# onolab-tmu/overiva

Hardware: AMD Instinct MI355X
Metric: AuxIVA iterations/sec (2048 bins x 4000 frames x 8 mics) (higher is better)
Workload: dtype f32

## Files before the change

include/overiva_hip.h:

```cpp
#ifndef OVERIVA_HIP_H
#define OVERIVA_HIP_H

#ifdef __cplusplus
extern "C" {
#endif

#define OIVA_OK 0
#define OIVA_ERR_ARG (-1)
#define OIVA_ERR_HIP (-2)
#define OIVA_ERR_STATE (-3)
#define OIVA_ERR_NUMERIC (-4)

#define OIVA_MODEL_LAPLACE 0
#define OIVA_MODEL_GAUSS 1

#define OIVA_MAX_CHANNELS 32

#define OIVA_PREC_FAST 0
#define OIVA_PREC_UPDATE_F64 1
#define OIVA_PREC_UPDATE_ROWS 2
#define OIVA_PREC_COV_F64 4
#define OIVA_PREC_PRECISE (OIVA_PREC_UPDATE_F64 | OIVA_PREC_COV_F64)

typedef struct oiva_plan oiva_plan;
// ... 28 lines not shown
int oiva_plan_demix_dev(oiva_plan *p, int proj_back, void **Y_dev);
int oiva_plan_demix_c128(oiva_plan *p, void *Y_host, long long row_pitch_bytes, int proj_back);

#define OIVA_XCHG_MAX_RANKS 16
#define OIVA_XCHG_HANDLE_BYTES 64
typedef struct oiva_xchg oiva_xchg;
int oiva_xchg_create(oiva_xchg **x, int device, int rank, int world, long long part_bytes);
int oiva_xchg_export(oiva_xchg *x, void *handle);
int oiva_xchg_connect(oiva_xchg *x, const void *handles);
int oiva_xchg_push(oiva_xchg *x, void *stream, const void *part_dev, long long part_bytes, int epoch);
int oiva_xchg_wait(oiva_xchg *x, void *stream, int epoch);
int oiva_xchg_gathered(oiva_xchg *x, int epoch, void **gathered);
int oiva_xchg_poll(oiva_xchg *x, int epoch, int timeout_ms, int *arrived);
int oiva_xchg_force(oiva_xchg *x, int epoch);
int oiva_xchg_destroy(oiva_xchg *x);

int oiva_plan_set_w_pca(oiva_plan *p, double *evals_host);
int oiva_plan_set_w_eig(oiva_plan *p);
int oiva_plan_get_w(oiva_plan *p, void *W_host, int f64);

int oiva_plan_sync(oiva_plan *p);
int oiva_plan_save_w(oiva_plan *p);
int oiva_plan_restore_w(oiva_plan *p);

int oiva_plan_iterate_timed(oiva_plan *p, int n, float *total_ms, float *per_kernel_ms);
#define OIVA_N_STAGES 4

int oiva_plan_get_cov_splits(oiva_plan *p, int *nsplit);
int oiva_plan_set_cov_splits(oiva_plan *p, int nsplit);
int oiva_plan_set_cov_quad(oiva_plan *p, int enable, int *active);
int oiva_plan_set_pow_splits(oiva_plan *p, int nsplit);
int oiva_plan_set_cov_hmfma(oiva_plan *p, int enable);
int oiva_plan_set_fuse_cov_update(oiva_plan *p, int enable, int *active);
int oiva_plan_use_graph(oiva_plan *p, int enable);
int oiva_plan_set_precision(oiva_plan *p, int flags);

struct oiva_xchg;
#define OIVA_RESIDENT_INFO 12
#define OIVA_RESIDENT_PHASES 8
int oiva_plan_set_resident(oiva_plan *p, int enable);
int oiva_plan_resident_info(oiva_plan *p, int *info );
int oiva_plan_resident_phases(oiva_plan *p, double *phase_us , int *n_iter);
int oiva_plan_resident_debug(oiva_plan *p, int timeout_ms, int stall_block);
int oiva_plan_resident_debug_from(oiva_plan *p, int timeout_ms, int stall_block, int first_stalled_iteration);
int oiva_plan_resident_loopback(oiva_plan *p, int world);
#define OIVA_RESIDENT_STAMPS 16
int oiva_plan_resident_trace(oiva_plan *p, int enable, unsigned long long *stamps_host, int *n_wg, int *n_iter);
int oiva_plan_resident_connect(oiva_plan *p, struct oiva_xchg *x);
int oiva_plan_fused_connect(oiva_plan *p, struct oiva_xchg *x);
int oiva_plan_fused_loopback(oiva_plan *p, int world);
int oiva_plan_fused_debug(oiva_plan *p, int timeout_ms, int stall);
int oiva_plan_set_resident_splits(oiva_plan *p, int nsplit);

int oiva_test_set_rinv(oiva_plan *p, const float *rinv_host );
int oiva_test_get_rinv(oiva_plan *p, float *rinv_host , float *wscale_host );
int oiva_test_run_weighted_cov(oiva_plan *p);
int oiva_test_get_v(oiva_plan *p, void *V_host , int f64);
int oiva_test_run_update(oiva_plan *p);
int oiva_test_get_what(oiva_plan *p, void *What_host , int f64);
int oiva_test_set_what(oiva_plan *p, const void *What_host, int f64);
int oiva_test_run_power(oiva_plan *p, float *p_host );
int oiva_test_time_stage(oiva_plan *p, int stage, int reps, float *avg_ms);

#define OIVA_OGIVE_DEMIX 0
#define OIVA_OGIVE_MIX 1
#define OIVA_OGIVE_SWITCHING 2
int oiva_plan_ogive_begin(oiva_plan *p, int update_mode, int model);
int oiva_plan_ogive_iterate(oiva_plan *p, int first_epoch, int n, double step_size, double tol, int *epochs_run,
                            int *converged, double *max_delta);

typedef struct oiva_batch oiva_batch;
int oiva_batch_create(oiva_batch **out, int device, int B, int T, int F, int M, int K, int model, void *stream);
int oiva_batch_destroy(oiva_batch *b);
int oiva_batch_set_x_host(oiva_batch *b, const void *X_host, int f64);
int oiva_batch_set_x_dev(oiva_batch *b, const void *X_dev);
int oiva_batch_covariance(oiva_batch *b);
int oiva_batch_set_w(oiva_batch *b, const void *W0_host, int f64);
int oiva_batch_set_w_eig(oiva_batch *b);
int oiva_batch_iterate(oiva_batch *b, int n);
int oiva_batch_demix(oiva_batch *b, void *Y_host, int f64, int proj_back);
int oiva_batch_get_w(oiva_batch *b, void *W_host, int f64);
int oiva_batch_status(oiva_batch *b, int *status);
int oiva_batch_time_stages(oiva_batch *b, int n, float *total_ms, float *per_stage_ms);

typedef int oiva_status;
oiva_status oiva_batch_get_cx(oiva_batch *b, void *Cx_host, int f64);
oiva_status oiva_batch_ogive_begin(oiva_batch *b, int update_mode, int model);
oiva_status oiva_batch_ogive_iterate(oiva_batch *b, int first_epoch, int n, double step_size, double tol, int *epochs_run,
                                     int *converged, double *max_delta);

oiva_status oiva_batch_create_ragged(oiva_batch **out, int device, int B, const int *frames, int F, int M, int K, int model,
                                     void *stream);

typedef struct oiva_stft oiva_stft;
// ... 23 lines not shown
```

overiva_amd/_lib.py:

```python
import ctypes as C
import os

import numpy as np

_PKG = os.path.dirname(os.path.abspath(__file__))
LIB_PATH = os.environ.get("OIVA_LIB") or os.path.join(_PKG, "liboveriva_hip.so")

OK, ERR_ARG, ERR_HIP, ERR_STATE, ERR_NUMERIC = 0, -1, -2, -3, -4
MODEL_IDS = {"laplace": 0, "gauss": 1}
N_STAGES = 4
PREC_FAST, PREC_UPDATE_F64, PREC_UPDATE_ROWS, PREC_COV_F64 = 0, 1, 2, 4
PREC_PRECISE = PREC_UPDATE_F64 | PREC_COV_F64
PREC_MIXED = PREC_UPDATE_F64
PREC_BY_NAME = {"fast": PREC_FAST, "mixed": PREC_MIXED, "precise": PREC_PRECISE}
STAGE_NAMES = ("demix_power", "activation", "weighted_cov", "ip_update")


class HipLibraryMissing(ImportError):
    pass


class HipError(RuntimeError):
    """a HIP runtime call failed inside the library"""

# ... 14 lines not shown
    "oiva_plan_set_w": [_vp, _vp, _i],
    "oiva_plan_iterate": [_vp, _i],
    "oiva_plan_power": [_vp],
    "oiva_plan_power_buffer": [_vp, _i, C.POINTER(_vp), C.POINTER(_ll)],
    "oiva_plan_update": [_vp, _vp, _i],
    "oiva_plan_demix": [_vp, _vp, _ll, _i],
    "oiva_plan_demix_dev": [_vp, _i, _vp],
    "oiva_plan_set_io_slab": [_vp, _ll],
    "oiva_host_prefault": [_vp, _ll],
    "oiva_pool_trim": [],
    "oiva_plan_demix_c128": [_vp, _vp, _ll, _i],
    "oiva_plan_set_w_pca": [_vp, _vp],
    "oiva_plan_set_w_eig": [_vp],
    "oiva_xchg_create": [_vp, _i, _i, _i, _ll],
    "oiva_xchg_export": [_vp, _vp],
    "oiva_xchg_connect": [_vp, _vp],
    "oiva_xchg_push": [_vp, _vp, _vp, _ll, _i],
    "oiva_xchg_wait": [_vp, _vp, _i],
    "oiva_xchg_gathered": [_vp, _i, _vp],
    "oiva_xchg_poll": [_vp, _i, _i, _vp],
    "oiva_xchg_force": [_vp, _i],
    "oiva_xchg_destroy": [_vp],
    "oiva_plan_get_w": [_vp, _vp, _i],
    "oiva_plan_sync": [_vp],
    "oiva_plan_save_w": [_vp],
    "oiva_plan_restore_w": [_vp],
    "oiva_plan_iterate_timed": [_vp, _i, _fp, _fp],
    "oiva_plan_get_cov_splits": [_vp, C.POINTER(_i)],
    "oiva_plan_set_cov_splits": [_vp, _i],
    "oiva_plan_set_cov_quad": [_vp, _i, C.POINTER(_i)],
    "oiva_plan_set_pow_splits": [_vp, _i],
    "oiva_plan_set_cov_hmfma": [_vp, _i],
    "oiva_plan_set_fuse_cov_update": [_vp, _i, C.POINTER(_i)],
    "oiva_plan_use_graph": [_vp, _i],
    "oiva_plan_set_precision": [_vp, _i],
    "oiva_plan_set_resident": [_vp, _i],
    "oiva_plan_resident_info": [_vp, C.POINTER(_i)],
    "oiva_plan_resident_phases": [_vp, C.POINTER(C.c_double), C.POINTER(_i)],
    "oiva_plan_resident_debug": [_vp, _i, _i],
    "oiva_plan_resident_debug_from": [_vp, _i, _i, _i],
    "oiva_plan_resident_loopback": [_vp, _i],
    "oiva_plan_fused_connect": [_vp, _vp],
    "oiva_plan_fused_loopback": [_vp, _i],
    "oiva_plan_fused_debug": [_vp, _i, _i],
    "oiva_plan_resident_connect": [_vp, _vp],
    "oiva_plan_resident_trace": [_vp, _i, _vp, C.POINTER(_i), C.POINTER(_i)],
    "oiva_plan_set_resident_splits": [_vp, _i],
    "oiva_test_set_rinv": [_vp, _vp],
    "oiva_test_get_rinv": [_vp, _vp, _vp],
    "oiva_test_run_weighted_cov": [_vp],
    "oiva_test_get_v": [_vp, _vp, _i],
    "oiva_test_run_update": [_vp],
    "oiva_test_get_what": [_vp, _vp, _i],
    "oiva_test_set_what": [_vp, _vp, _i],
    "oiva_test_run_power": [_vp, _vp],
    "oiva_test_time_stage": [_vp, _i, _i, _fp],
    "oiva_plan_ogive_begin": [_vp, _i, _i],
    "oiva_plan_ogive_iterate": [_vp, _i, _i, C.c_double, C.c_double, C.POINTER(_i), C.POINTER(_i), C.POINTER(C.c_double)],
    "oiva_batch_create": [C.POINTER(_vp), _i, _i, _i, _i, _i, _i, _i, _vp],
    "oiva_batch_destroy": [_vp],
    "oiva_batch_set_x_host": [_vp, _vp, _i],
    "oiva_batch_set_x_dev": [_vp, _vp],
    "oiva_batch_covariance": [_vp],
    "oiva_batch_set_w": [_vp, _vp, _i],
    "oiva_batch_set_w_eig": [_vp],
    "oiva_batch_iterate": [_vp, _i],
    "oiva_batch_demix": [_vp, _vp, _i, _i],
    "oiva_batch_get_w": [_vp, _vp, _i],
    "oiva_batch_status": [_vp, C.POINTER(_i)],
    "oiva_batch_time_stages": [_vp, _i, _fp, _fp],
    "oiva_batch_get_cx": [_vp, _vp, _i],
    "oiva_batch_ogive_begin": [_vp, _i, _i],
    "oiva_batch_ogive_iterate": [_vp, _i, _i, C.c_double, C.c_double, C.POINTER(_i), C.POINTER(_i), C.POINTER(C.c_double)],
    "oiva_batch_create_ragged": [C.POINTER(_vp), _i, _i, C.POINTER(_i), _i, _i, _i, _i, _vp],
    "oiva_stft_create": [C.POINTER(_vp), _i, _i, _i, _i, _i, _vp, _vp],
    "oiva_stft_destroy": [_vp],
    "oiva_stft_shape": [_vp, C.POINTER(_i), C.POINTER(_i)],
    "oiva_stft_analysis": [_vp, _vp, _vp, C.POINTER(_vp)],
    "oiva_stft_synthesis": [_vp, _vp, _i, _vp],
    "oiva_bstft_create": [C.POINTER(_vp), _i, _i, C.POINTER(_i), _i, _i, _i, _vp, _vp, _vp],
    "oiva_bstft_destroy": [_vp],
    "oiva_bstft_shape": [_vp, C.POINTER(_i), C.POINTER(_i)],
    "oiva_bstft_analysis": [_vp, _vp, C.POINTER(_vp)],
    "oiva_bstft_synthesis_dev": [_vp, _vp, _i, _vp],
    "oiva_bstft_phase_ms": [_vp, _fp],
    "oiva_batch_demix_dev": [_vp, _i, C.POINTER(_vp)],
    "oiva_device_to_host": [_vp, _vp, _ll],
}
# ... 88 lines not shown
```

overiva_amd/csrc/kernels_demix.hip:

```cpp
#include "oiva_device.h"
#include "demix_arith.h"

namespace oiva {
namespace {

constexpr int kPowUnroll = 2;

template <int M, int KP>
__global__ __launch_bounds__(kBlock) void power_kernel(const float2* __restrict__ X, const float2* __restrict__ What,
                                                       float* __restrict__ Ppart, int T, int F, int K, int tcp) {
    extern __shared__ __attribute__((aligned(16))) float sp[];
    const int tid = threadIdx.x;
    const int lane = tid & 63;
    const int wave = tid >> 6;
    const int b = lane & 15;
    const int q = lane >> 4;
    const int f = (blockIdx.x * kWaves + wave) * kBinsPerWave + b;
    const bool fvalid = f < F;
    const int fc = fvalid ? f : F - 1;
    const int k0 = blockIdx.z * KP;
    const int t_begin = blockIdx.y * tcp;
    const int t_end = min(T, t_begin + tcp);
    const int len = t_end - t_begin;
    const int nsteps = (len + 3) >> 2;

    float wr[KP][M], wi[KP][M];
    load_wconj<M, KP>(What, fc, k0, K, wr, wi);

    const size_t frame_stride = (size_t)F * M;
    const float2* pbase = X + (size_t)fc * M;
    for (int i = 0; i < nsteps; i += kPowUnroll) {
        float xr[kPowUnroll][M], xi[kPowUnroll][M];
#pragma unroll
        for (int u = 0; u < kPowUnroll; ++u) {
            const int tl = 4 * (i + u) + q;
            const int t = tl < len ? t_begin + tl : T - 1;
            load_x<M>(pbase + (size_t)t * frame_stride, xr[u], xi[u]);
        }
#pragma unroll
        for (int u = 0; u < kPowUnroll; ++u) {
            const int tl = 4 * (i + u) + q;
            const bool live = tl < len;
#pragma unroll
            for (int kk = 0; kk < KP; ++kk) {
                float yr, yi;
                demix_one<M>(wr[kk], wi[kk], xr[u], xi[u], yr, yi);
                float pw = fmaf(yr, yr, yi * yi);
                pw = fvalid ? pw : 0.f;
                pw = row16_sum(pw);
                if (b == 0 && live) sp[(wave * tcp + tl) * KP + kk] = pw;
            }
        }
    }
    __syncthreads();
    for (int e = tid; e < len * KP; e += kBlock) {
        const int tl = e / KP, kk = e - tl * KP;
        float s = sp[(0 * tcp + tl) * KP + kk];
#pragma unroll
        for (int w = 1; w < kWaves; ++w) s += sp[(w * tcp + tl) * KP + kk];
        if (k0 + kk < K) Ppart[((size_t)blockIdx.x * T + t_begin + tl) * K + k0 + kk] = s;
    }
}

template <int M, int KP>
// ... 82 lines not shown
                if (sd > 0.) {
                    zr = (float)(sr / sd);
                    zi = (float)(si / sd);
                }
#pragma unroll
                for (int m = 0; m < M; ++m) {
                    const float a = wr[kk][m], c = wi[kk][m];
                    wr[kk][m] = a * zr + c * zi;
                    wi[kk][m] = c * zr - a * zi;
                }
            }
        }
    }
    const size_t frame_stride = (size_t)F * M;
    const float2* px = X + ((size_t)(t_begin + q) * F + f) * M;
    for (int t = t_begin + q; t < t_end; t += 16) {
        float xr[M], xi[M];
        load_x<M>(px, xr, xi);
#pragma unroll
        for (int kk = 0; kk < KP; ++kk) {
            float yr, yi;
            demix_one<M>(wr[kk], wi[kk], xr, xi, yr, yi);
            if (k0 + kk < K) Y[((size_t)t * F + f) * K + k0 + kk] = make_float2(yr, yi);
        }
        px += 16 * frame_stride;
    }
}

template <int M, int KP>
hipError_t launch_power_one(hipStream_t s, const float2* X, const float2* What, float* Ppart, int T, int F, int K,
                            const PowGeom& g) {
    dim3 grid(g.nb, g.nsplit, (K + KP - 1) / KP);
    const size_t shmem = (size_t)kWaves * g.tcp * KP * sizeof(float);
    hipLaunchKernelGGL((power_kernel<M, KP>), grid, dim3(kBlock), shmem, s, X, What, Ppart, T, F, K, g.tcp);
    return hipGetLastError();
}

template <int M, int KP>
hipError_t launch_stats_one(hipStream_t s, const float2* X, const float2* What, float* Spart, int T, int F, int K,
                            const CovGeom& g) {
    dim3 grid(g.nbg, g.nsplit, (K + KP - 1) / KP);
    hipLaunchKernelGGL((stats_kernel<M, KP>), grid, dim3(kBlock), 0, s, X, What, Spart, T, F, K, g.tc);
    return hipGetLastError();
}

template <int M, int KP>
hipError_t launch_write_one(hipStream_t s, const float2* X, const float2* What, const float* Spart, int nsplit,
                            float2* Y, int T, int F, int K) {
    const int tc = 256;
    dim3 grid((F + kBinsPerWave - 1) / kBinsPerWave, (T + tc - 1) / tc, (K + KP - 1) / KP);
    hipLaunchKernelGGL((write_kernel<M, KP>), grid, dim3(kBlock), 0, s, X, What, Spart, nsplit, Y, T, F, K, tc);
    return hipGetLastError();
}

#define OIVA_DISPATCH_M(CALL)            \
    switch (M) {                         \
        case 1: CALL(1); break;          \
        case 2: CALL(2); break;          \
        case 3: CALL(3); break;          \
        case 4: CALL(4); break;          \
        case 5: CALL(5); break;          \
        case 6: CALL(6); break;          \
        case 7: CALL(7); break;          \
        case 8: CALL(8); break;          \
        case 9: CALL(9); break;          \
        case 10: CALL(10); break;        \
        case 11: CALL(11); break;        \
// ... 59 lines not shown
```

overiva_amd/csrc/oiva_internal.h:

```cpp
#pragma once
#include <hip/hip_runtime.h>
#include <hip/hip_ext.h>

#include <string>

#include "overiva_hip.h"

namespace oiva {

constexpr int kNarrowMax = 16;
constexpr int kWideMax = OIVA_MAX_CHANNELS;

int fail_with(int code, const std::string& msg);
int xchg_peers(oiva_xchg* x, char** peers, int* rank, int* world, size_t* slot_bytes);

constexpr int kBinsPerWave = 16;
constexpr int kPhasesPerWave = 4;
constexpr int kBlock = 256;
constexpr int kWaves = kBlock / 64;

__host__ __device__ inline int herm_pair_index(int M, int c, int d) {
    return M + 2 * (c * M - (c * (c + 1)) / 2 + (d - c - 1));
}

// ... 5 lines not shown

struct KernelTimer {
    hipEvent_t start = nullptr, stop = nullptr;
};
KernelTimer& kernel_timer();
inline void arm_kernel_timer(hipEvent_t start, hipEvent_t stop) {
    kernel_timer().start = start;
    kernel_timer().stop = stop;
}
template <typename Kern, typename... Args>
hipError_t launch_dominant(Kern kernel, dim3 grid, dim3 block, size_t shmem, hipStream_t s, Args... args) {
    KernelTimer& t = kernel_timer();
    if (t.start != nullptr) {
        hipExtLaunchKernelGGL(kernel, grid, block, (unsigned)shmem, s, t.start, t.stop, 0, args...);
        t.start = t.stop = nullptr;
    } else {
        hipLaunchKernelGGL(kernel, grid, block, shmem, s, args...);
    }
    return hipGetLastError();
}

struct CovGeom {
    int nsplit;
    int tc;
    int kc;
    int nbg;
    int hmfma = 0;
    int half16 = 0;
    int pair32 = 0;
    int pad = 0;
    int quad = 0;
    int part32 = 0;
};
struct PowGeom {
    int nb;
    int nsplit;
    int tcp;
    int kp;
};
constexpr int kPowMaxFrames = 512;

hipError_t launch_cov(hipStream_t s, const float2* X, const float2* Xpad, const float* R, float* Wt, float* wscale, int model, int raw,
                      void* Vpart, bool f64, int T, int F, int M, int K, const CovGeom& g);
hipError_t launch_pad_channels(hipStream_t s, const float2* X, float2* Xpad, long long n_tf, int M);
hipError_t launch_cov_mfma(hipStream_t s, const float2* X, const float* R, float* Wt, float* wscale, int model, int raw,
                           void* Vpart, bool f64, int T, int F, int M, int K, int nsplit, int tc);
bool cov_quad_supported(int M, int K);
int cov_quad_sources_per_pass(int K);
hipError_t launch_cov_quad(hipStream_t s, const float2* X, const float* R, float* Wt, float* wscale, int model, int raw,
                           double* Vpart, int T, int F, int M, int Mv, int K, const CovGeom& g);
hipError_t launch_cov_weights(hipStream_t s, const float* R, float* Wt, float* wscale, int model, int raw, int T, int K, int Kp);
bool cov_pair64_supported(int M);
int cov_pair64_sources_per_pass(int K);
int cov_pair64_bins_per_block();
hipError_t launch_cov_pair64(hipStream_t s, const float2* X, const float* R, float* Wt, float* wscale, int model, int raw,
                             double* Vpart, int T, int F, int M, int K, const CovGeom& g);
bool cov_pair32_supported(int M, int K);
int cov_pair32_sources_per_pass();
int cov_pair32_bins_per_block();
hipError_t launch_cov_pair32(hipStream_t s, const float2* X, const float* R, float* Wt, float* wscale, int model, int raw,
                             double* Vpart, int T, int F, int M, int K, const CovGeom& g);
bool cov_half16_supported(int M, int K);
int cov_half16_sources_per_pass(int K);
hipError_t launch_cov_half16(hipStream_t s, const float2* X, const float* R, float* Wt, float* wscale, int model, int raw,
                             double* Vpart, int T, int F, int M, int Mv, int K, const CovGeom& g);
bool cov_hmfma_supported(int M, int K);
hipError_t launch_cov_hmfma(hipStream_t s, const float2* X, const float* Wt, double* Vpart, int T, int F, int M, int Mv, int K, const CovGeom& g);
bool cov_hmfma64_supported(int M, int K);
hipError_t launch_cov_hmfma64(hipStream_t s, const float2* X, const double* Wt, double* Vpart, int T, int F, int M, int Mv, int K, const CovGeom& g);
bool cov_half16_f64_supported(int M, int K);
int cov_half16_f64_sources_per_pass(int K);
hipError_t launch_cov_half16_f64(hipStream_t s, const float2* X, const float* R, float* Wt, float* wscale, int model, int raw,
                                 double* Vpart, int T, int F, int M, int Mv, int K, const CovGeom& g);
// ... 212 lines not shown
```

overiva_amd/csrc/plan.hip:

```cpp
#include <algorithm>
#include <cmath>
#include <cstdint>
#include <cstdlib>
#include <cstring>
#include <mutex>
#include <string>
#include <vector>

#include "host_io.h"
#include "oiva_internal.h"
#include "resident.h"

using namespace oiva;

namespace {

thread_local std::string g_err;

int fail(int code, const std::string& msg) {
    g_err = msg;
    return code;
}

}
// ... 105 lines not shown
}
}

struct oiva_plan {
    int device = 0;
    int T = 0, F = 0, M = 0, K = 0, model = 0, F_total = 0;
    hipStream_t stream = nullptr;
    bool own_stream = false;

    const float2* X = nullptr;
    float2* X_owned = nullptr;
    size_t x_owned_bytes = 0, y_bytes = 0;
    float2* X_pad = nullptr;
    float2* What = nullptr;
    double2* What64 = nullptr;
    bool what64_valid = false;
    double* Cx = nullptr;
    void* Vpart = nullptr;
    float* Ppart = nullptr;
    int ppart_alloc = 0;
    float* Plocal = nullptr;
    void* Wwide = nullptr;
    float* R = nullptr;
    float* wscale = nullptr;
    float* Spart = nullptr;
    float2* Y = nullptr;
    double2* scratch_c = nullptr;
    double* scratch_p = nullptr;

    CovGeom cov{};
    bool cov_quad_on = true;
    bool cov_hmfma_on = true;
    bool fuse_cov_update = false;
    CovGeom stg{};
    PowGeom pw{};
    int n_cu = 256;
    int vpart_splits_alloc = 0;

    bool have_x = false, have_cx = false, have_w = false;
    bool pad_valid = false;
    bool wscale_pending = false;
    int raw_weights = 0;
    int prec = 0;
    bool upd_f64() const { return prec & OIVA_PREC_UPDATE_F64; }
    bool cov_f64() const { return prec & OIVA_PREC_COV_F64; }
    bool vpart_f64() const { return vpart_f64_of(cov); }
    bool vpart_f64_of(const CovGeom& g) const { return cov_f64() || M <= 8 || M > kNarrowMax || g.quad || (g.half16 && !g.part32); }
    int use_graph = 0;
    OgiveState og{};
    std::vector<void*> og_bufs;
    bool og_ready = false;
    int og_mode = 0, og_model = 0;
    hipGraphExec_t og_graph = nullptr;
    int og_graph_n = 0, og_graph_phase = -1;
    double og_graph_mu = 0., og_graph_tol = 0.;
    ResidentGeom rg{};
    bool res_ok = false;
    bool res_on = false;
    void* res_block = nullptr;
    float* res_parts = nullptr;
    float* res_psum = nullptr;
    double* res_vpart = nullptr;
    double* res_rsum = nullptr;
    float2* res_wpub = nullptr;
    unsigned* res_flags = nullptr;
    float2* res_what = nullptr;
// ... 145 lines not shown
        return;
    }
    g.nbg = ceil_div(p->F, kBinsPerWave);
    g.kc = 2;
    const int nz = ceil_div(p->K, g.kc);
    const int nsplit = std::min(16, pick_splits(p->n_cu * 4, g.nbg * nz, p->T, 128));
    g.tc = round_up(ceil_div(p->T, nsplit), 16);
    g.nsplit = ceil_div(p->T, g.tc);
    p->stg = g;
}

void choose_pow_geom(oiva_plan* p, int nsplit_req) {
    PowGeom g;
    g.nb = ceil_div(p->F, kBinsPerWave * kWaves);
    if (p->M > kNarrowMax) {
        g.kp = wide_pow_sources_per_pass(p->K);
        const int groups = g.nb * ceil_div(p->K, g.kp);
        const int nsplit = nsplit_req > 0 ? nsplit_req : pick_splits(p->n_cu * 4, groups, p->T, 16);
        g.tcp = round_up(ceil_div(p->T, nsplit), 4);
        g.nsplit = ceil_div(p->T, g.tcp);
        p->pw = g;
        return;
    }
    g.kp = pow_sources_per_pass(p->M, p->K);
    int nsplit = nsplit_req;
    if (nsplit <= 0) {
        const int per_cu_x12 = (g.kp == 1 && p->M <= 8) ? 24 : 12;
        nsplit = pick_splits(std::max(p->n_cu / 2, p->n_cu * per_cu_x12 / std::max(p->M, 1)), g.nb, p->T, 32);
    }
    int tcp = round_up(ceil_div(p->T, nsplit), 4);
    tcp = std::min(std::max(tcp, 4), kPowMaxFrames);
    g.tcp = tcp;
    g.nsplit = ceil_div(p->T, tcp);
    p->pw = g;
}

int drop_graph(oiva_plan* p) {
    while (!p->graphs.empty()) {
        hipGraphExec_t g = p->graphs.back().second;
        p->graphs.pop_back();
        HIP_TRY(hipGraphExecDestroy(g));
    }
    if (p->og_graph) {
        HIP_TRY(hipGraphExecDestroy(p->og_graph));
        p->og_graph = nullptr;
    }
    return OIVA_OK;
}

size_t vpart_floats(const oiva_plan* p, int nsplit) { return (size_t)nsplit * p->F * p->K * p->M * p->M; }

int ensure_vpart(oiva_plan* p) {
    if (p->cov.nsplit > p->vpart_splits_alloc) {
        if (p->Vpart) HIP_TRY(hipFree(p->Vpart));
        p->Vpart = nullptr;
        HIP_TRY(dev_malloc(&p->Vpart, (vpart_floats(p, p->cov.nsplit) + 2) * sizeof(double)));
        p->vpart_splits_alloc = p->cov.nsplit;
    }
    return OIVA_OK;
}

int stage_power(oiva_plan* p) {
    HIP_TRY(launch_power(p->stream, p->X, p->X_pad && p->pad_valid ? p->X_pad : nullptr, p->What, p->Ppart, p->T, p->F, p->M, p->K, p->pw));
    return OIVA_OK;
}
int stage_activation(oiva_plan* p, const float* parts, int nparts) {
    if (p->fx_on && parts == p->Ppart) {
        HIP_TRY(launch_activation_xchg(p->stream, parts, nparts, p->fx_gath, p->fx_rank, p->fx_world, p->fx_loopback ? (p->fx_stall ? 2 : 1) : 0, p->fx_nblk_own, p->fx_nblk_peer, p->fx_state + 16,
                                       p->fx_state, (long long)(p->fx_timeout_ms > 0 ? p->fx_timeout_ms : 2000) * 100000, p->R, p->T, p->K,
                                       p->model, p->F_total));
        p->raw_weights = 0;
        return OIVA_OK;
    }
    HIP_TRY(launch_activation(p->stream, parts, nparts, p->R, p->T, p->K, p->model, p->F_total));
    p->raw_weights = 0;
    return OIVA_OK;
}
int stage_cov(oiva_plan* p) {
    HIP_TRY(launch_cov(p->stream, p->X, p->X_pad, p->R, p->Wwide ? static_cast<float*>(p->Wwide) : p->Plocal , p->wscale, p->model,
                       p->raw_weights, p->Vpart, p->cov_f64(), p->T, p->F, p->M, p->K, p->cov));
    p->wscale_pending = !p->raw_weights;
    return OIVA_OK;
}
int stage_update(oiva_plan* p, bool init_only) {
    UpdateArgs a;
    a.What = p->What;
    a.What64 = p->upd_f64() ? p->What64 : nullptr;
    a.Cx = p->Cx;
    a.Vpart = p->Vpart;
    a.vpart_f64 = p->vpart_f64() ? 1 : 0;
    a.wscale = (!init_only && p->wscale_pending) ? p->wscale : nullptr;
    a.nsplit = p->cov.nsplit;
    a.T = p->T;
    a.F = p->F;
    a.M = p->M;
    a.K = p->K;
// ... 288 lines not shown
    p->T = T;
    p->F = F;
    p->M = M;
    p->K = K;
    p->model = model;
    p->F_total = F_total;
    if (stream) {
        p->stream = (hipStream_t)stream;
    } else {
        hipError_t e = hipStreamCreateWithFlags(&p->stream, hipStreamNonBlocking);
        if (e != hipSuccess) {
            delete p;
            return fail(OIVA_ERR_HIP, std::string("hipStreamCreate: ") + hipGetErrorString(e));
        }
        p->own_stream = true;
    }
    {
        hipDeviceProp_t prop;
        if (hipGetDeviceProperties(&prop, device) == hipSuccess && prop.multiProcessorCount > 0)
            p->n_cu = prop.multiProcessorCount;
    }
    if (M > 8 && M <= kNarrowMax && M % 2 == 1) {
        hipError_t ep = dev_malloc((void**)&p->X_pad, (size_t)T * F * (M + 1) * sizeof(float2));
        if (ep != hipSuccess) {
            oiva_plan_destroy(p);
            return fail(OIVA_ERR_HIP, std::string("allocation of the padded copy of X failed: ") + hipGetErrorString(ep));
        }
    }
    {
        const char* v = std::getenv("OIVA_COV_HMFMA");
        p->cov_hmfma_on = !(v && v[0] == '0');
        const char* u = std::getenv("OIVA_COV_UPDATE");
        p->fuse_cov_update = u && u[0] == '1';
    }
    choose_cov_geom(p, 0);
    choose_pow_geom(p, 0);
    choose_stats_geom(p);
    p->res_ok = resident_geometry(T, F, M, K, p->n_cu, 0, &p->rg);
    const size_t nTK = (size_t)T * K;
    const size_t nFMM = (size_t)F * M * M;
    hipError_t e = hipSuccess;
    auto alloc = [&](void** ptr, size_t bytes) {
        if (e == hipSuccess) e = dev_malloc(ptr, bytes);
    };
    alloc((void**)&p->What, nFMM * sizeof(float2));
    alloc((void**)&p->What64, nFMM * sizeof(double2));
    alloc((void**)&p->Cx, nFMM * sizeof(double));
    alloc((void**)&p->Ppart, (size_t)p->pw.nb * nTK * sizeof(float));
    p->ppart_alloc = p->pw.nb;
    alloc((void**)&p->Plocal, std::max(nTK, ((size_t)T + 1) * 32) * sizeof(float));
    if (M > kNarrowMax) alloc((void**)&p->Wwide, nTK * sizeof(double));
    alloc((void**)&p->R, r_buffer_bytes(T, K));
    if (e == hipSuccess) e = hipMemset(p->R, 0, r_buffer_bytes(T, K));
    alloc((void**)&p->wscale, (size_t)K * sizeof(float));
    alloc((void**)&p->Spart, (size_t)p->stg.nsplit * F * K * 3 * sizeof(float));
    alloc((void**)&p->scratch_c, (size_t)K * nFMM * sizeof(double2));
    alloc((void**)&p->scratch_p, std::max((size_t)K * nFMM, nTK) * sizeof(double));
    for (auto& ev : p->ev) {
        if (e == hipSuccess) e = hipEventCreate(&ev);
    }
    if (e != hipSuccess) {
        oiva_plan_destroy(p);
        return fail(OIVA_ERR_HIP, std::string("allocation failed: ") + hipGetErrorString(e));
    }
    int rc = ensure_vpart(p);
    if (rc) {
// ... 708 lines not shown
    DeviceGuard guard(p->device);
    if (enable >= 0) {
        HIP_TRY(hipStreamSynchronize(p->stream));
        int rc = drop_graph(p);
        if (rc) return rc;
        p->fuse_cov_update = enable != 0;
    }
    if (active) *active = cov_update_applies(p) ? 1 : 0;
    return OIVA_OK;
}

int oiva_plan_set_cov_hmfma(oiva_plan* p, int enable) {
    NEED(p, OIVA_ERR_ARG, "null plan");
    DeviceGuard guard(p->device);
    HIP_TRY(hipStreamSynchronize(p->stream));
    int rc = drop_graph(p);
    if (rc) return rc;
    p->cov_hmfma_on = enable != 0;
    choose_cov_geom(p, 0);
    return ensure_vpart(p);
}

int oiva_plan_set_pow_splits(oiva_plan* p, int nsplit) {
    NEED(p, OIVA_ERR_ARG, "null plan");
    NEED(nsplit >= 0 && nsplit <= p->T, OIVA_ERR_ARG, "bad split count");
    DeviceGuard guard(p->device);
    HIP_TRY(hipStreamSynchronize(p->stream));
    int rc = drop_graph(p);
    if (rc) return rc;
    choose_pow_geom(p, nsplit);
    return OIVA_OK;
}

int oiva_plan_use_graph(oiva_plan* p, int enable) {
    NEED(p, OIVA_ERR_ARG, "null plan");
    DeviceGuard guard(p->device);
    p->use_graph = enable ? 1 : 0;
    if (!enable) return drop_graph(p);
    if (p->have_x && p->have_cx && p->have_w && (p->F == p->F_total || p->fx_on)) return build_graphs(p);
    return OIVA_OK;
}

int oiva_plan_set_precision(oiva_plan* p, int flags) {
    NEED(p, OIVA_ERR_ARG, "null plan");
    NEED((flags & ~(OIVA_PREC_UPDATE_F64 | OIVA_PREC_UPDATE_ROWS | OIVA_PREC_COV_F64)) == 0, OIVA_ERR_ARG, "unknown precision flag");
    DeviceGuard guard(p->device);
    HIP_TRY(hipStreamSynchronize(p->stream));
    int rc = drop_graph(p);
    if (rc) return rc;
    if ((flags & OIVA_PREC_UPDATE_F64) && p->have_w && !p->what64_valid) {
        std::vector<double2> wh;
        if ((rc = download_what(p, wh)) || (rc = upload_what(p, wh))) return rc;
    }
    const bool cov_changed = ((flags ^ p->prec) & (OIVA_PREC_COV_F64 | ((p->M > 8 || p->cov.pair32) ? OIVA_PREC_UPDATE_F64 : 0))) != 0;
    p->prec = flags;
    if (cov_changed) {
        choose_cov_geom(p, 0);
        if ((rc = ensure_vpart(p))) return rc;
    }
    return OIVA_OK;
}

int oiva_plan_set_resident(oiva_plan* p, int enable) {
    NEED(p, OIVA_ERR_ARG, "null plan");
    if (!enable) {
        p->res_on = false;
// ... 360 lines not shown
            case 0: return stage_power(p);
            case 1: return stage_activation(p, p->Ppart, p->pw.nb);
            case 2: return cov_update_applies(p) ? stage_cov_update(p) : stage_cov(p);
            default: return cov_update_applies(p) ? OIVA_OK : stage_update(p, false);
        }
    };
    if ((rc = run())) return rc;
    HIP_TRY(hipEventRecord(p->ev[0], p->stream));
    for (int i = 0; i < reps; ++i)
        if ((rc = run())) return rc;
    HIP_TRY(hipEventRecord(p->ev[1], p->stream));
    HIP_TRY(hipEventSynchronize(p->ev[1]));
    float ms = 0.f;
    HIP_TRY(hipEventElapsedTime(&ms, p->ev[0], p->ev[1]));
    *avg_ms = ms / reps;
    return OIVA_OK;
}

int oiva_test_run_power(oiva_plan* p, float* p_host) {
    NEED(p && p_host, OIVA_ERR_ARG, "null argument");
    NEED(p->have_x && p->have_w, OIVA_ERR_STATE, "X / W not set");
    DeviceGuard guard(p->device);
    int rc = stage_power(p);
    if (rc) return rc;
    const size_t n = (size_t)p->T * p->K;
    HIP_TRY(launch_sum_parts(p->stream, p->Ppart, false, p->pw.nb, p->scratch_p, (long long)n, 1.));
    HIP_TRY(hipStreamSynchronize(p->stream));
    std::vector<double> sum(n);
    HIP_TRY(hipMemcpy(sum.data(), p->scratch_p, n * sizeof(double), hipMemcpyDeviceToHost));
    for (size_t i = 0; i < n; ++i) p_host[i] = (float)sum[i];
    return OIVA_OK;
}

}
```

overiva_amd/plan.py:

```python
import ctypes as C

import numpy as np

from . import _lib


def _is_f64(a):
    if a.dtype == np.complex128:
        return 1
    if a.dtype == np.complex64:
        return 0
    raise TypeError(f"complex64 or complex128 expected, got {a.dtype}")


class DeviceX:

    def __init__(self, ptr, shape, owner=None, host_dtype=np.complex64):
        self.ptr = int(ptr)
        self.shape = tuple(int(v) for v in shape)
        self.owner = owner
        self.dtype = np.dtype(host_dtype)
        self.ndim = 3


# ... 147 lines not shown
    def sync(self):
        _lib.check(self.lib.oiva_plan_sync(self.h))

    def save_w(self):
        _lib.check(self.lib.oiva_plan_save_w(self.h))

    def restore_w(self):
        _lib.check(self.lib.oiva_plan_restore_w(self.h))

    def cov_splits(self):
        n = C.c_int()
        _lib.check(self.lib.oiva_plan_get_cov_splits(self.h, C.byref(n)))
        return n.value

    def set_cov_splits(self, n):
        _lib.check(self.lib.oiva_plan_set_cov_splits(self.h, int(n)))

    def set_cov_quad(self, enable=True):
        a = C.c_int()
        _lib.check(self.lib.oiva_plan_set_cov_quad(self.h, 1 if enable else 0, C.byref(a)))
        return bool(a.value)

    def set_cov_hmfma(self, enable=True):
        _lib.check(self.lib.oiva_plan_set_cov_hmfma(self.h, 1 if enable else 0))

    def set_fuse_cov_update(self, enable=True):
        a = C.c_int()
        _lib.check(self.lib.oiva_plan_set_fuse_cov_update(self.h, -1 if enable is None else (1 if enable else 0), C.byref(a)))
        return bool(a.value)

    def set_pow_splits(self, n):
        _lib.check(self.lib.oiva_plan_set_pow_splits(self.h, int(n)))

    def use_graph(self, enable=True):
        _lib.check(self.lib.oiva_plan_use_graph(self.h, 1 if enable else 0))

    def set_precision(self, mode="fast", row_layout=False):
        flags = _lib.PREC_BY_NAME[mode] if isinstance(mode, str) else int(mode)
        if row_layout:
            flags |= _lib.PREC_UPDATE_ROWS
        _lib.check(self.lib.oiva_plan_set_precision(self.h, flags))

    RESIDENT_INFO = ("qualifies", "enabled", "bin_groups", "frame_splits", "frames_per_split", "frames_per_lane",
                     "frames_in_registers", "lds_bytes", "last_give_up_code", "launches", "fallbacks", "x_bytes_per_cu")
    RESIDENT_PHASES = ("demix_power", "parts", "activation", "cov_accumulate", "cov_reduce", "wait_partials", "ip_update", "wait_w")

    def set_resident(self, enable=True):
        _lib.check(self.lib.oiva_plan_set_resident(self.h, 1 if enable else 0))

    def resident_info(self):
        arr = (C.c_int * len(self.RESIDENT_INFO))()
        _lib.check(self.lib.oiva_plan_resident_info(self.h, arr))
        return dict(zip(self.RESIDENT_INFO, list(arr)))

    def resident_phases(self):
        arr = (C.c_double * len(self.RESIDENT_PHASES))()
        n = C.c_int()
        _lib.check(self.lib.oiva_plan_resident_phases(self.h, arr, C.byref(n)))
        return dict(zip(self.RESIDENT_PHASES, list(arr))), n.value

    def set_resident_splits(self, nsplit=0):
        _lib.check(self.lib.oiva_plan_set_resident_splits(self.h, int(nsplit)))

    def resident_connect(self, xchg_handle):
        _lib.check(self.lib.oiva_plan_resident_connect(self.h, xchg_handle))

# ... 29 lines not shown
    def t_get_rinv(self):
        r = np.empty((self.T, self.K), np.float32)
        w = np.empty((self.K,), np.float32)
        _lib.check(self.lib.oiva_test_get_rinv(self.h, _lib.ptr(r), _lib.ptr(w)))
        return r, w

    def t_run_weighted_cov(self):
        _lib.check(self.lib.oiva_test_run_weighted_cov(self.h))

    def t_get_v(self, dtype=np.complex64):
        v = np.empty((self.K, self.F, self.M, self.M), dtype)
        _lib.check(self.lib.oiva_test_get_v(self.h, _lib.ptr(v), _is_f64(v)))
        return v

    def t_run_update(self):
        _lib.check(self.lib.oiva_test_run_update(self.h))

    def t_get_what(self, dtype=np.complex64):
        w = np.empty((self.F, self.M, self.M), dtype)
        _lib.check(self.lib.oiva_test_get_what(self.h, _lib.ptr(w), _is_f64(w)))
        return w

    def t_set_what(self, What):
        What = np.asarray(What)
        What = np.ascontiguousarray(What, dtype=np.complex64 if What.dtype == np.complex64 else np.complex128)
        assert What.shape == (self.F, self.M, self.M)
        _lib.check(self.lib.oiva_test_set_what(self.h, _lib.ptr(What), _is_f64(What)))

    def t_time_stage(self, stage, reps=20):
        ms = C.c_float()
        _lib.check(self.lib.oiva_test_time_stage(self.h, _lib.STAGE_NAMES.index(stage), int(reps), C.byref(ms)))
        return ms.value

    def t_run_power(self):
        p = np.empty((self.T, self.K), np.float32)
        _lib.check(self.lib.oiva_test_run_power(self.h, _lib.ptr(p)))
        return p
```

Before: 4958.

## Reverse power-kernel frame traversal to reuse cache from preceding covariance pass

```diff
diff --git a/include/overiva_hip.h b/include/overiva_hip.h
--- a/include/overiva_hip.h
+++ b/include/overiva_hip.h
@@ -84,6 +84,7 @@
 int oiva_plan_set_pow_splits(oiva_plan *p, int nsplit);
 int oiva_plan_set_cov_hmfma(oiva_plan *p, int enable);
 int oiva_plan_set_fuse_cov_update(oiva_plan *p, int enable, int *active);
+int oiva_plan_set_power_reverse(oiva_plan *p, int enable);
 int oiva_plan_use_graph(oiva_plan *p, int enable);
 int oiva_plan_set_precision(oiva_plan *p, int flags);
 
@@ -112,6 +113,8 @@
 int oiva_test_get_what(oiva_plan *p, void *What_host , int f64);
 int oiva_test_set_what(oiva_plan *p, const void *What_host, int f64);
 int oiva_test_run_power(oiva_plan *p, float *p_host );
+int oiva_test_get_ppart(oiva_plan *p, float *parts_host, int *nparts);
+int oiva_test_power_order(int nsplit, int tcp, int cov_splits, int cov_tc, int *order);
 int oiva_test_time_stage(oiva_plan *p, int stage, int reps, float *avg_ms);
 
 #define OIVA_OGIVE_DEMIX 0
diff --git a/overiva_amd/_lib.py b/overiva_amd/_lib.py
--- a/overiva_amd/_lib.py
+++ b/overiva_amd/_lib.py
@@ -70,6 +70,7 @@
     "oiva_plan_set_pow_splits": [_vp, _i],
     "oiva_plan_set_cov_hmfma": [_vp, _i],
     "oiva_plan_set_fuse_cov_update": [_vp, _i, C.POINTER(_i)],
+    "oiva_plan_set_power_reverse": [_vp, _i],
     "oiva_plan_use_graph": [_vp, _i],
     "oiva_plan_set_precision": [_vp, _i],
     "oiva_plan_set_resident": [_vp, _i],
@@ -92,6 +93,8 @@
     "oiva_test_get_what": [_vp, _vp, _i],
     "oiva_test_set_what": [_vp, _vp, _i],
     "oiva_test_run_power": [_vp, _vp],
+    "oiva_test_get_ppart": [_vp, _vp, C.POINTER(_i)],
+    "oiva_test_power_order": [_i, _i, _i, _i, C.POINTER(_i)],
     "oiva_test_time_stage": [_vp, _i, _i, _fp],
     "oiva_plan_ogive_begin": [_vp, _i, _i],
     "oiva_plan_ogive_iterate": [_vp, _i, _i, C.c_double, C.c_double, C.POINTER(_i), C.POINTER(_i), C.POINTER(C.c_double)],
diff --git a/overiva_amd/csrc/kernels_demix.hip b/overiva_amd/csrc/kernels_demix.hip
--- a/overiva_amd/csrc/kernels_demix.hip
+++ b/overiva_amd/csrc/kernels_demix.hip
@@ -8,7 +8,7 @@
 
 template <int M, int KP>
 __global__ __launch_bounds__(kBlock) void power_kernel(const float2* __restrict__ X, const float2* __restrict__ What,
-                                                       float* __restrict__ Ppart, int T, int F, int K, int tcp) {
+                                                       float* __restrict__ Ppart, int T, int F, int K, int tcp, int rev, PowOrder ord) {
     extern __shared__ __attribute__((aligned(16))) float sp[];
     const int tid = threadIdx.x;
     const int lane = tid & 63;
@@ -19,17 +19,20 @@
     const bool fvalid = f < F;
     const int fc = fvalid ? f : F - 1;
     const int k0 = blockIdx.z * KP;
-    const int t_begin = blockIdx.y * tcp;
+    const int chunk = ord.cs > 0 ? power_chunk_tail_first(blockIdx.y, gridDim.y, ord) : (int)blockIdx.y;
+    const int t_begin = chunk * tcp;
     const int t_end = min(T, t_begin + tcp);
     const int len = t_end - t_begin;
     const int nsteps = (len + 3) >> 2;
+    const int ngroups = (nsteps + kPowUnroll - 1) / kPowUnroll;
 
     float wr[KP][M], wi[KP][M];
     load_wconj<M, KP>(What, fc, k0, K, wr, wi);
 
     const size_t frame_stride = (size_t)F * M;
     const float2* pbase = X + (size_t)fc * M;
-    for (int i = 0; i < nsteps; i += kPowUnroll) {
+    for (int g = 0; g < ngroups; ++g) {
+        const int i = (rev ? ngroups - 1 - g : g) * kPowUnroll;
         float xr[kPowUnroll][M], xi[kPowUnroll][M];
 #pragma unroll
         for (int u = 0; u < kPowUnroll; ++u) {
@@ -178,7 +181,7 @@
                             const PowGeom& g) {
     dim3 grid(g.nb, g.nsplit, (K + KP - 1) / KP);
     const size_t shmem = (size_t)kWaves * g.tcp * KP * sizeof(float);
-    hipLaunchKernelGGL((power_kernel<M, KP>), grid, dim3(kBlock), shmem, s, X, What, Ppart, T, F, K, g.tcp);
+    hipLaunchKernelGGL((power_kernel<M, KP>), grid, dim3(kBlock), shmem, s, X, What, Ppart, T, F, K, g.tcp, g.rev, g.ord);
     return hipGetLastError();
 }
 
diff --git a/overiva_amd/csrc/oiva_internal.h b/overiva_amd/csrc/oiva_internal.h
--- a/overiva_amd/csrc/oiva_internal.h
+++ b/overiva_amd/csrc/oiva_internal.h
@@ -61,13 +61,44 @@
     int quad = 0;
     int part32 = 0;
 };
+constexpr int kPowOrderMaxSplits = 64;
+struct PowOrder {
+    int cs = 0;
+    int q = 0;
+    int first[kPowOrderMaxSplits + 1] = {};
+};
+inline PowOrder make_pow_order(int n, int tcp, int cs, int ctc) {
+    PowOrder o;
+    if (cs < 1 || cs > kPowOrderMaxSplits || ctc < 1 || tcp < 1 || n < 1) return o;
+    o.cs = cs;
+    for (int s = 0; s < cs; ++s) {
+        const long long c = (long long)s * ctc / tcp;
+        o.first[s] = c < n ? (int)c : n;
+    }
+    o.first[cs] = n;
+    o.q = n;
+    for (int s = 0; s < cs; ++s) o.q = o.first[s + 1] - o.first[s] < o.q ? o.first[s + 1] - o.first[s] : o.q;
+    return o;
+}
+__host__ __device__ inline int power_chunk_tail_first(int y, int n, const PowOrder& o) {
+    if (y < o.q * o.cs) return o.first[y % o.cs + 1] - 1 - y / o.cs;
+    y -= o.q * o.cs;
+    for (int r = o.q; r < n; ++r)
+        for (int s = 0; s < o.cs; ++s)
+            if (o.first[s + 1] - o.first[s] > r && y-- == 0) return o.first[s + 1] - 1 - r;
+    return n - 1;
+}
 struct PowGeom {
     int nb;
     int nsplit;
     int tcp;
     int kp;
+    int rev = 0;
+    PowOrder ord{};
+    int rounds = 1;
 };
 constexpr int kPowMaxFrames = 512;
+
 
 hipError_t launch_cov(hipStream_t s, const float2* X, const float2* Xpad, const float* R, float* Wt, float* wscale, int model, int raw,
                       void* Vpart, bool f64, int T, int F, int M, int K, const CovGeom& g);
diff --git a/overiva_amd/csrc/plan.hip b/overiva_amd/csrc/plan.hip
--- a/overiva_amd/csrc/plan.hip
+++ b/overiva_amd/csrc/plan.hip
@@ -161,6 +161,7 @@
     bool cov_quad_on = true;
     bool cov_hmfma_on = true;
     bool fuse_cov_update = false;
+    int power_reverse = 1;
     CovGeom stg{};
     PowGeom pw{};
     int n_cu = 256;
@@ -372,6 +373,10 @@
     tcp = std::min(std::max(tcp, 4), kPowMaxFrames);
     g.tcp = tcp;
     g.nsplit = ceil_div(p->T, tcp);
+    int bpc = 0;
+    if (p->M <= 8 || p->K <= 4)
+        if (pow_blocks_per_cu(p->M, g.kp, g.tcp, &bpc) == hipSuccess && bpc > 0)
+            g.rounds = (int)ceil_div((long long)g.nb * g.nsplit * ceil_div(p->K, g.kp), (long long)bpc * p->n_cu);
     p->pw = g;
 }
 
@@ -401,7 +406,12 @@
 }
 
 int stage_power(oiva_plan* p) {
-    HIP_TRY(launch_power(p->stream, p->X, p->X_pad && p->pad_valid ? p->X_pad : nullptr, p->What, p->Ppart, p->T, p->F, p->M, p->K, p->pw));
+    PowGeom g = p->pw;
+    if (p->power_reverse) {
+        g.rev = 1;
+        if (g.rounds > 1 || p->power_reverse > 1) g.ord = make_pow_order(g.nsplit, g.tcp, p->cov.nsplit, p->cov.tc);
+    }
+    HIP_TRY(launch_power(p->stream, p->X, p->X_pad && p->pad_valid ? p->X_pad : nullptr, p->What, p->Ppart, p->T, p->F, p->M, p->K, g));
     return OIVA_OK;
 }
 int stage_activation(oiva_plan* p, const float* parts, int nparts) {
@@ -756,6 +766,8 @@
         p->cov_hmfma_on = !(v && v[0] == '0');
         const char* u = std::getenv("OIVA_COV_UPDATE");
         p->fuse_cov_update = u && u[0] == '1';
+        const char* r = std::getenv("OIVA_POWER_REVERSE");
+        p->power_reverse = (r && r[0] == '0') ? 0 : (r && r[0] == '2') ? 2 : 1;
     }
     choose_cov_geom(p, 0);
     choose_pow_geom(p, 0);
@@ -1530,6 +1542,16 @@
     return OIVA_OK;
 }
 
+int oiva_plan_set_power_reverse(oiva_plan* p, int enable) {
+    NEED(p, OIVA_ERR_ARG, "null plan");
+    DeviceGuard guard(p->device);
+    HIP_TRY(hipStreamSynchronize(p->stream));
+    int rc = drop_graph(p);
+    if (rc) return rc;
+    p->power_reverse = enable < 0 ? 0 : enable > 2 ? 2 : enable;
+    return OIVA_OK;
+}
+
 int oiva_plan_use_graph(oiva_plan* p, int enable) {
     NEED(p, OIVA_ERR_ARG, "null plan");
     DeviceGuard guard(p->device);
@@ -1956,4 +1978,22 @@
     return OIVA_OK;
 }
 
-}
+int oiva_test_get_ppart(oiva_plan* p, float* parts_host, int* nparts) {
+    NEED(p && nparts, OIVA_ERR_ARG, "null argument");
+    *nparts = p->pw.nb;
+    if (!parts_host) return OIVA_OK;
+    DeviceGuard guard(p->device);
+    HIP_TRY(hipStreamSynchronize(p->stream));
+    HIP_TRY(hipMemcpy(parts_host, p->Ppart, (size_t)p->pw.nb * p->T * p->K * sizeof(float), hipMemcpyDeviceToHost));
+    return OIVA_OK;
+}
+
+int oiva_test_power_order(int nsplit, int tcp, int cov_splits, int cov_tc, int* order) {
+    NEED(order && nsplit >= 1 && tcp >= 1 && cov_splits >= 1 && cov_tc >= 1, OIVA_ERR_ARG, "bad arguments");
+    NEED(cov_splits <= kPowOrderMaxSplits, OIVA_ERR_ARG, "more covariance splits than the order table holds");
+    const PowOrder o = make_pow_order(nsplit, tcp, cov_splits, cov_tc);
+    for (int y = 0; y < nsplit; ++y) order[y] = power_chunk_tail_first(y, nsplit, o);
+    return OIVA_OK;
+}
+
+}
diff --git a/overiva_amd/plan.py b/overiva_amd/plan.py
--- a/overiva_amd/plan.py
+++ b/overiva_amd/plan.py
@@ -203,6 +203,9 @@
     def set_pow_splits(self, n):
         _lib.check(self.lib.oiva_plan_set_pow_splits(self.h, int(n)))
 
+    def set_power_reverse(self, enable=True):
+        _lib.check(self.lib.oiva_plan_set_power_reverse(self.h, int(enable)))
+
     def use_graph(self, enable=True):
         _lib.check(self.lib.oiva_plan_use_graph(self.h, 1 if enable else 0))
 
@@ -298,6 +301,13 @@
         _lib.check(self.lib.oiva_test_time_stage(self.h, _lib.STAGE_NAMES.index(stage), int(reps), C.byref(ms)))
         return ms.value
 
+    def t_get_ppart(self):
+        n = C.c_int()
+        _lib.check(self.lib.oiva_test_get_ppart(self.h, None, C.byref(n)))
+        out = np.empty((n.value, self.T, self.K), np.float32)
+        _lib.check(self.lib.oiva_test_get_ppart(self.h, _lib.ptr(out), C.byref(n)))
+        return out
+
     def t_run_power(self):
         p = np.empty((self.T, self.K), np.float32)
         _lib.check(self.lib.oiva_test_run_power(self.h, _lib.ptr(p)))
```

After: 5118, median of 6. +3.2%, better.
